# vlongle/pixie

Hardware: AMD Instinct MI355X
Metric: voxels/s (128^3 U-Net fwd) + MPM particle-steps/s (higher is better)
Workload: dtype f32 (operands split fp16 hi+lo, 3 f16 MFMAs/product, fp32 accumulate); 1 GPU; 128^3x64 feature grid -> SegmentationUNet+RegressionUNet forward (+argmax/one-hot combine), 1 scene per GPU per step; grid=128, feature_channels=64, parallelism=scene-parallel x1, executor=c+hip_graph

## Files before the change

### pixie_amd/csrc/conv3d_f16x3.hip

```cpp
#include <hip/hip_runtime.h>

#include <cstdlib>
#include <map>
#include <string>
#include <type_traits>

#include "../../include/pixie_hip.h"
#include "common.h"

namespace pixie {

typedef float f32x16 __attribute__((ext_vector_type(16)));
typedef _Float16 f16x8 __attribute__((ext_vector_type(8)));

constexpr int kW16HeaderU4 = 4;

struct Conv16Args {
    const float* in0; const float* in1;
    int c0, cin;
    int ID, IH, IW;
    int LD, LH, LW;
    int ups;
    int stride;
    int OD, OH, OW;
    const float* pro_a; const float* pro_b; const float* gamma; const float* beta;
    int act;
    const uint4* w16;
    const float* wf;
    const float* bias;
    int cout, coutp;
    const float* residual; float* out;
    const unsigned* amax0; const unsigned* amax1;
    float in_bound;
    int TX, TY, TZ, lTX, lTY;
    int tiles_x, tiles_y, tiles_z, n_tiles;
    int HX, HY, HZ, HYX, CS;
    unsigned mHX, mHYX;
    float* stats; unsigned* out_amax;
    float* partial; int chunks_per_slice;
    int epi_lds;
    const float* sk_in0; const float* sk_in1;
    int sk_c0, sk_cin;
    const uint4* sk_w16; const float* sk_bias;
    const unsigned* sk_amax0; const unsigned* sk_amax1;
};

__device__ __forceinline__ int fast_div16(int n, int d, unsigned magic) {
    return (d == 1) ? n : (int)__umulhi((unsigned)n, magic);
}
__device__ __forceinline__ float act16(float t, int act) {
    if (act == 1) return t > 0.0f ? t : 0.02f * t;
    if (act == 2) return t / (1.0f + __expf(-t));
    return t;
}
__device__ __forceinline__ int scale_exponent(float bound) {
    const unsigned bits = __float_as_uint(bound);
    const int eb = (int)((bits >> 23) & 0xffu) - 127;
    if (!(bound > 0.0f) || eb > 100) return 0;
    int e = 14 - eb;
    return e > 100 ? 100 : (e < -100 ? -100 : e);
}
__device__ __forceinline__ float pow2i(int e) { return __uint_as_float((unsigned)(e + 127) << 23); }

template <int KS, int MB, int NB, bool EX = false, bool SP = false>
__device__ __forceinline__ void conv3d_f16x3_body(const Conv16Args& A) {
    static_assert(!SP || (KS == 3 && NB == 4 && !EX), "sub-pixel path: 3^3, two x parities x two voxel blocks per wave");
    extern __shared__ uint4 smem16[];
    constexpr int PAD = (KS == 3) ? 1 : 0;
    constexpr int NW = 4, NT = 64 * NW;
    const int bufsz = 4 * A.CS;

    const int tid = threadIdx.x;
    const int lane = tid & 63;
    const int wave = tid >> 6;
    const int kh = lane >> 5;
    const int l31 = lane & 31;

    int t = blockIdx.x;
    {
        const int per = (A.n_tiles + 7) >> 3;
        const int cand = (t & 7) * per + (t >> 3);
        if ((A.n_tiles & 7) == 0) t = cand;
    }
    int par = 0;
    if constexpr (SP) { par = t & 3; t >>= 2; }
    const int py = par & 1, pz = par >> 1;
    const int tx = t % A.tiles_x; t /= A.tiles_x;
    const int ty = t % A.tiles_y;
    const int tz = t / A.tiles_y;
    const int ox0 = tx * A.TX, oy0 = ty * A.TY, oz0 = tz * A.TZ;
    const int cout0 = blockIdx.y * (MB * 32);
    const int lx0 = SP ? ox0 - 1 : ox0 * A.stride - PAD;
    const int ly0 = SP ? oy0 - 1 + py : oy0 * A.stride - PAD;
    const int lz0 = SP ? oz0 - 1 + pz : oz0 * A.stride - PAD;
    const size_t ISP = (size_t)A.ID * A.IH * A.IW;
    const size_t OSP = (size_t)A.OD * A.OH * A.OW;

    int voff[NB];
    int ovox[NB];
    bool valid[NB];
#pragma unroll
    for (int nb = 0; nb < NB; ++nb) {
        if constexpr (SP) {
            const int px = nb >> 1;
            const int j = (wave * 2 + (nb & 1)) * 32 + l31;
            int x = j & (A.TX - 1);
            int y = (j >> A.lTX) & (A.TY - 1);
            int z = j >> (A.lTX + A.lTY);
            const int gx = 2 * (ox0 + x) + px, gy = 2 * (oy0 + y) + py, gz = 2 * (oz0 + z) + pz;
            const bool v = (z < A.TZ) && (gx < A.OW) && (gy < A.OH) && (gz < A.OD);
            if (!v) { x = 0; y = 0; z = 0; }
            voff[nb] = (z * A.HY + y) * A.HX + x + px + kh * A.CS;
            ovox[nb] = v ? (gz * A.OH + gy) * A.OW + gx : 0;
            valid[nb] = v;
            continue;
        }
        const int j = (wave * NB + nb) * 32 + l31;
        int x = j & (A.TX - 1);
        int y = (j >> A.lTX) & (A.TY - 1);
        int z = j >> (A.lTX + A.lTY);
        const bool v = (z < A.TZ) && (ox0 + x < A.OW) && (oy0 + y < A.OH) && (oz0 + z < A.OD);
        if (!v) { x = 0; y = 0; z = 0; }
        voff[nb] = ((z * A.HY + y) * A.HX + x) * A.stride + kh * A.CS;
        ovox[nb] = ((oz0 + z) * A.OH + (oy0 + y)) * A.OW + ox0 + x;
        valid[nb] = v;
    }

    float bound = A.in_bound;
    if (A.amax0) {
        bound = __uint_as_float(*A.amax0);
        if (A.amax1) bound = fmaxf(bound, __uint_as_float(*A.amax1));
    }
    const int ex = EX ? 0 : scale_exponent(bound);
    const float sx = pow2i(ex);

    f32x16 acc[MB][NB];
#pragma unroll
    for (int mb = 0; mb < MB; ++mb)
#pragma unroll
        for (int nb = 0; nb < NB; ++nb)
#pragma unroll
            for (int r = 0; r < 16; ++r) acc[mb][nb][r] = 0.0f;

    const int KG = A.cin >> 3;
    const size_t tap_stride = (size_t)KG * A.coutp;
    const size_t plane = (size_t)(SP ? 64 : KS * KS * KS) * tap_stride;
    const uint4* wHi = A.w16 + kW16HeaderU4 + (size_t)kh * A.coutp + cout0 + l31 + (size_t)(par * 16) * tap_stride;
    const uint4* wLo = wHi + plane;
    const float* wF = A.wf + (size_t)kh * A.coutp + cout0 + l31;

    constexpr int TAPS = KS * KS * KS;
    auto stage_chunk = [&](int c_base, uint4* buf, int stid, int nthr) {
        uint4* bHi = buf;
        uint4* bLo = buf + 2 * A.CS;
        float pa[16], pb[16];
        {
            float pv = 0.0f;
            if (A.pro_a) pv = (lane & 16) ? A.pro_b[c_base + (lane & 15)] : A.pro_a[c_base + (lane & 15)];
#pragma unroll
            for (int j = 0; j < 16; ++j) {
                pa[j] = __int_as_float(__builtin_amdgcn_readlane(__float_as_int(pv), j));
                pb[j] = __int_as_float(__builtin_amdgcn_readlane(__float_as_int(pv), 16 + j));
            }
        }
        const bool has_aff = A.gamma != nullptr;
        for (int v0 = stid; v0 < A.CS; v0 += 2 * nthr) {
            float val[2][16];
            float gm[2], bt[2];
            int sidx[2];
            bool ok[2];
#pragma unroll
            for (int u = 0; u < 2; ++u) {
                const int vox = v0 + u * nthr;
                int rem = vox;
                const int hz = fast_div16(rem, A.HYX, A.mHYX);
                rem -= hz * A.HYX;
                const int hy = fast_div16(rem, A.HX, A.mHX);
                const int hx = rem - hy * A.HX;
                const int lz = lz0 + hz, ly = ly0 + hy, lx = lx0 + hx;
                ok[u] = vox < A.CS && (unsigned)lz < (unsigned)A.LD && (unsigned)ly < (unsigned)A.LH && (unsigned)lx < (unsigned)A.LW;
                sidx[u] = ok[u] ? ((lz >> A.ups) * A.IH + (ly >> A.ups)) * A.IW + (lx >> A.ups) : 0;
            }
#pragma unroll
            for (int u = 0; u < 2; ++u) {
#pragma unroll
                for (int j = 0; j < 16; ++j) {
                    const int cg = c_base + j;
                    const float* src = (cg < A.c0) ? (A.in0 + (size_t)cg * ISP) : (A.in1 + (size_t)(cg - A.c0) * ISP);
                    val[u][j] = src[sidx[u]];
                }
                gm[u] = 1.0f; bt[u] = 0.0f;
                if (has_aff) { gm[u] = A.gamma[sidx[u]]; bt[u] = A.beta[sidx[u]]; }
            }
            auto convert = [&](auto has_pro, auto act_c) {
#pragma unroll
                for (int u = 0; u < 2; ++u) {
                    const int vox = v0 + u * nthr;
                    if (EX) {
                        float* bF = reinterpret_cast<float*>(buf);
#pragma unroll
                        for (int j = 0; j < 16; ++j) {
                            float t = val[u][j];
                            if (decltype(has_pro)::value) t = t * pa[j] + pb[j];
                            t = t * gm[u] + bt[u];
                            const float sc = ok[u] ? act16(t, decltype(act_c)::value) : 0.0f;
                            if (vox < A.CS) bF[j * A.CS + vox] = sc;
                        }
                        continue;
                    }
                    f16x8 vh[2], vl[2];
#pragma unroll
                    for (int j = 0; j < 16; ++j) {
                        float t = val[u][j];
                        if (decltype(has_pro)::value) t = t * pa[j] + pb[j];
                        t = t * gm[u] + bt[u];
                        const float sc = ok[u] ? act16(t, decltype(act_c)::value) * sx : 0.0f;
                        const _Float16 h = (_Float16)sc;
                        vh[j >> 3][j & 7] = h;
                        vl[j >> 3][j & 7] = (_Float16)(sc - (float)h);
                    }
                    if (vox < A.CS) {
                        bHi[vox] = __builtin_bit_cast(uint4, vh[0]);
                        bHi[A.CS + vox] = __builtin_bit_cast(uint4, vh[1]);
                        bLo[vox] = __builtin_bit_cast(uint4, vl[0]);
                        bLo[A.CS + vox] = __builtin_bit_cast(uint4, vl[1]);
                    }
                }
            };
            using T = std::true_type; using F = std::false_type;
            if (A.pro_a) {
                if (A.act == 1) convert(T{}, std::integral_constant<int, 1>{});
                else if (A.act == 2) convert(T{}, std::integral_constant<int, 2>{});
                else convert(T{}, std::integral_constant<int, 0>{});
            } else {
                if (A.act == 1) convert(F{}, std::integral_constant<int, 1>{});
                else if (A.act == 2) convert(F{}, std::integral_constant<int, 2>{});
                else convert(F{}, std::integral_constant<int, 0>{});
            }
        }
    };
    auto mfma_chunk = [&](int c_base, const uint4* buf) {
        __builtin_amdgcn_s_setprio(3);
        if constexpr (EX) {
            const float* ldsF = reinterpret_cast<const float*>(buf);
            const size_t tapw = (size_t)A.cin * A.coutp;
            const float* wc = wF + (size_t)c_base * A.coutp;
            float a[8][MB], an[8][MB];
#pragma unroll
            for (int kp = 0; kp < 8; ++kp)
#pragma unroll
                for (int mb = 0; mb < MB; ++mb) a[kp][mb] = wc[(size_t)(2 * kp) * A.coutp + mb * 32];
#pragma unroll 1
            for (int zy = 0; zy < KS * KS; ++zy) {
                const int dz = zy / KS, dy = zy - dz * KS;
                const int rowoff = (dz * A.HY + dy) * A.HX;
#pragma unroll
                for (int dx = 0; dx < KS; ++dx) {
                    const int tap = zy * KS + dx;
                    const int nxt = (tap + 1 < TAPS) ? tap + 1 : tap;
#pragma unroll
                    for (int kp = 0; kp < 8; ++kp)
#pragma unroll
                        for (int mb = 0; mb < MB; ++mb) an[kp][mb] = wc[(size_t)nxt * tapw + (size_t)(2 * kp) * A.coutp + mb * 32];
                    __builtin_amdgcn_sched_barrier(0);
#pragma unroll
                    for (int kp = 0; kp < 8; ++kp) {
                        float b[NB];
#pragma unroll
                        for (int nb = 0; nb < NB; ++nb) b[nb] = ldsF[voff[nb] + rowoff + dx + 2 * kp * A.CS];
#pragma unroll
                        for (int mb = 0; mb < MB; ++mb)
#pragma unroll
                            for (int nb = 0; nb < NB; ++nb)
                                acc[mb][nb] = __builtin_amdgcn_mfma_f32_32x32x2f32(a[kp][mb], b[nb], acc[mb][nb], 0, 0, 0);
                    }
#pragma unroll
                    for (int kp = 0; kp < 8; ++kp)
#pragma unroll
                        for (int mb = 0; mb < MB; ++mb) a[kp][mb] = an[kp][mb];
                }
            }
            __builtin_amdgcn_s_setprio(0);
            return;
        }
        const uint4* ldsHi = buf;
        const uint4* ldsLo = buf + 2 * A.CS;
        const uint4* wh = wHi + (size_t)(c_base >> 3) * A.coutp;
        const uint4* wl = wLo + (size_t)(c_base >> 3) * A.coutp;
        if constexpr (SP) {
            f16x8 ah[MB], al[MB];
#pragma unroll
            for (int mb = 0; mb < MB; ++mb) {
                ah[mb] = __builtin_bit_cast(f16x8, wh[mb * 32]);
                al[mb] = __builtin_bit_cast(f16x8, wl[mb * 32]);
            }
#pragma unroll 1
            for (int zy = 0; zy < 4; ++zy) {
                const int rowoff = ((zy >> 1) * A.HY + (zy & 1)) * A.HX;
                const int zyn = zy < 3 ? zy + 1 : 3;
#pragma unroll
                for (int q = 0; q < 4; ++q) {
                    const int ex = q >> 1, px = q & 1;
                    const size_t nxt = (q < 3) ? (size_t)(((q + 1) & 1) * 8 + zy * 2 + ((q + 1) >> 1)) * tap_stride : (size_t)(zyn * 2) * tap_stride;
                    f16x8 ahn[MB], aln[MB];
#pragma unroll
                    for (int mb = 0; mb < MB; ++mb) {
                        ahn[mb] = __builtin_bit_cast(f16x8, wh[nxt + mb * 32]);
                        aln[mb] = __builtin_bit_cast(f16x8, wl[nxt + mb * 32]);
                    }
                    __builtin_amdgcn_sched_barrier(0);
                    f16x8 bh[2], bl[2];
#pragma unroll
                    for (int s = 0; s < 2; ++s) {
                        bh[s] = __builtin_bit_cast(f16x8, ldsHi[voff[px * 2 + s] + rowoff + ex]);
                        bl[s] = __builtin_bit_cast(f16x8, ldsLo[voff[px * 2 + s] + rowoff + ex]);
                    }
#pragma unroll
                    for (int mb = 0; mb < MB; ++mb)
#pragma unroll
                        for (int s = 0; s < 2; ++s)
                            acc[mb][px * 2 + s] = __builtin_amdgcn_mfma_f32_32x32x16_f16(al[mb], bh[s], acc[mb][px * 2 + s], 0, 0, 0);
#pragma unroll
                    for (int mb = 0; mb < MB; ++mb)
#pragma unroll
                        for (int s = 0; s < 2; ++s)
                            acc[mb][px * 2 + s] = __builtin_amdgcn_mfma_f32_32x32x16_f16(ah[mb], bl[s], acc[mb][px * 2 + s], 0, 0, 0);
#pragma unroll
                    for (int mb = 0; mb < MB; ++mb)
#pragma unroll
                        for (int s = 0; s < 2; ++s)
                            acc[mb][px * 2 + s] = __builtin_amdgcn_mfma_f32_32x32x16_f16(ah[mb], bh[s], acc[mb][px * 2 + s], 0, 0, 0);
#pragma unroll
                    for (int mb = 0; mb < MB; ++mb) { ah[mb] = ahn[mb]; al[mb] = aln[mb]; }
                }
            }
            __builtin_amdgcn_s_setprio(0);
            return;
        }
        f16x8 ah[MB], al[MB];
#pragma unroll
        for (int mb = 0; mb < MB; ++mb) {
            ah[mb] = __builtin_bit_cast(f16x8, wh[mb * 32]);
            al[mb] = __builtin_bit_cast(f16x8, wl[mb * 32]);
        }
#pragma unroll 1
        for (int zy = 0; zy < KS * KS; ++zy) {
            const int dz = zy / KS, dy = zy - dz * KS;
            const int rowoff = (dz * A.HY + dy) * A.HX;
#pragma unroll
            for (int dx = 0; dx < KS; ++dx) {
                const int tap = zy * KS + dx;
                const int nxt = (tap + 1 < TAPS) ? tap + 1 : tap;
                f16x8 ahn[MB], aln[MB];
#pragma unroll
                for (int mb = 0; mb < MB; ++mb) {
                    ahn[mb] = __builtin_bit_cast(f16x8, wh[(size_t)nxt * tap_stride + mb * 32]);
                    aln[mb] = __builtin_bit_cast(f16x8, wl[(size_t)nxt * tap_stride + mb * 32]);
                }
                __builtin_amdgcn_sched_barrier(0);
                f16x8 bh[NB], bl[NB];
#pragma unroll
                for (int nb = 0; nb < NB; ++nb) {
                    bh[nb] = __builtin_bit_cast(f16x8, ldsHi[voff[nb] + rowoff + dx]);
                    bl[nb] = __builtin_bit_cast(f16x8, ldsLo[voff[nb] + rowoff + dx]);
                }
#pragma unroll
                for (int mb = 0; mb < MB; ++mb)
#pragma unroll
                    for (int nb = 0; nb < NB; ++nb)
                        acc[mb][nb] = __builtin_amdgcn_mfma_f32_32x32x16_f16(al[mb], bh[nb], acc[mb][nb], 0, 0, 0);
#pragma unroll
                for (int mb = 0; mb < MB; ++mb)
#pragma unroll
                    for (int nb = 0; nb < NB; ++nb)
                        acc[mb][nb] = __builtin_amdgcn_mfma_f32_32x32x16_f16(ah[mb], bl[nb], acc[mb][nb], 0, 0, 0);
#pragma unroll
                for (int mb = 0; mb < MB; ++mb)
#pragma unroll
                    for (int nb = 0; nb < NB; ++nb)
                        acc[mb][nb] = __builtin_amdgcn_mfma_f32_32x32x16_f16(ah[mb], bh[nb], acc[mb][nb], 0, 0, 0);
#pragma unroll
                for (int mb = 0; mb < MB; ++mb) { ah[mb] = ahn[mb]; al[mb] = aln[mb]; }
            }
        }
        __builtin_amdgcn_s_setprio(0);
    };

    float inv2 = 0.0f;
    {
        const int c_begin = A.partial ? (int)blockIdx.z * A.chunks_per_slice * 16 : 0;
        const int c_end = A.partial ? min(A.cin, c_begin + A.chunks_per_slice * 16) : A.cin;
        for (int c_base = c_begin; c_base < c_end; c_base += 16) {
            __syncthreads();
            stage_chunk(c_base, smem16, tid, NT);
            __syncthreads();
            mfma_chunk(c_base, smem16);
        }
        if (!EX && !SP && A.sk_w16) {
            float sb = __uint_as_float(*A.sk_amax0);
            if (A.sk_amax1) sb = fmaxf(sb, __uint_as_float(*A.sk_amax1));
            const int ex2 = scale_exponent(sb);
            const float sx2 = pow2i(ex2);
            const float inv_main = __uint_as_float(A.w16[0].x) * pow2i(-ex);
            inv2 = __uint_as_float(A.sk_w16[0].x) * pow2i(-ex2);
            const float ratio = inv_main / inv2;
#pragma unroll
            for (int mb = 0; mb < MB; ++mb)
#pragma unroll
                for (int nb = 0; nb < NB; ++nb)
#pragma unroll
                    for (int r = 0; r < 16; ++r) acc[mb][nb][r] *= ratio;
            const int KG2 = A.sk_cin >> 3;
            const uint4* w2Hi = A.sk_w16 + kW16HeaderU4 + (size_t)kh * A.coutp + cout0 + l31;
            const uint4* w2Lo = w2Hi + (size_t)KG2 * A.coutp;
            const int centre = (KS == 3) ? (A.HY + 1) * A.HX + 1 : 0;
            const int tvox = A.TX * A.TY * A.TZ;
            for (int c2 = 0; c2 < A.sk_cin; c2 += 16) {
                f16x8 ah[MB], al[MB];
#pragma unroll
                for (int mb = 0; mb < MB; ++mb) {
                    ah[mb] = __builtin_bit_cast(f16x8, w2Hi[(size_t)(c2 >> 3) * A.coutp + mb * 32]);
                    al[mb] = __builtin_bit_cast(f16x8, w2Lo[(size_t)(c2 >> 3) * A.coutp + mb * 32]);
                }
                __syncthreads();
                uint4* bHi = smem16;
                uint4* bLo = smem16 + 2 * A.CS;
                for (int j = tid; j < tvox; j += NT) {
                    const int x = j & (A.TX - 1), y = (j >> A.lTX) & (A.TY - 1), z = j >> (A.lTX + A.lTY);
                    const bool okv = (ox0 + x < A.OW) && (oy0 + y < A.OH) && (oz0 + z < A.OD);
                    const size_t sidx = okv ? ((size_t)(oz0 + z) * A.IH + (oy0 + y)) * A.IW + ox0 + x : 0;
                    float val[16];
#pragma unroll
                    for (int q = 0; q < 16; ++q) {
                        const int cg = c2 + q;
                        const float* src = (cg < A.sk_c0) ? (A.sk_in0 + (size_t)cg * ISP) : (A.sk_in1 + (size_t)(cg - A.sk_c0) * ISP);
                        val[q] = src[sidx];
                    }
                    f16x8 vh[2], vl[2];
#pragma unroll
                    for (int q = 0; q < 16; ++q) {
                        const float sc = okv ? val[q] * sx2 : 0.0f;
                        const _Float16 hq = (_Float16)sc;
                        vh[q >> 3][q & 7] = hq;
                        vl[q >> 3][q & 7] = (_Float16)(sc - (float)hq);
                    }
                    const int slot = (z * A.HY + y) * A.HX + x + centre;
                    bHi[slot] = __builtin_bit_cast(uint4, vh[0]);
                    bHi[A.CS + slot] = __builtin_bit_cast(uint4, vh[1]);
                    bLo[slot] = __builtin_bit_cast(uint4, vl[0]);
                    bLo[A.CS + slot] = __builtin_bit_cast(uint4, vl[1]);
                }
                __syncthreads();
                f16x8 bh[NB], bl[NB];
#pragma unroll
                for (int nb = 0; nb < NB; ++nb) {
                    bh[nb] = __builtin_bit_cast(f16x8, bHi[voff[nb] + centre]);
                    bl[nb] = __builtin_bit_cast(f16x8, bLo[voff[nb] + centre]);
                }
#pragma unroll
                for (int mb = 0; mb < MB; ++mb)
#pragma unroll
                    for (int nb = 0; nb < NB; ++nb)
                        acc[mb][nb] = __builtin_amdgcn_mfma_f32_32x32x16_f16(al[mb], bh[nb], acc[mb][nb], 0, 0, 0);
#pragma unroll
                for (int mb = 0; mb < MB; ++mb)
#pragma unroll
                    for (int nb = 0; nb < NB; ++nb)
                        acc[mb][nb] = __builtin_amdgcn_mfma_f32_32x32x16_f16(ah[mb], bl[nb], acc[mb][nb], 0, 0, 0);
#pragma unroll
                for (int mb = 0; mb < MB; ++mb)
#pragma unroll
                    for (int nb = 0; nb < NB; ++nb)
                        acc[mb][nb] = __builtin_amdgcn_mfma_f32_32x32x16_f16(ah[mb], bh[nb], acc[mb][nb], 0, 0, 0);
            }
        }
    }

    const float inv = EX ? 1.0f : (A.sk_w16 ? inv2 : __uint_as_float(A.w16[0].x) * pow2i(-ex));
    if (A.partial) {
        float* dst = A.partial + (size_t)blockIdx.z * A.cout * OSP;
#pragma unroll
        for (int mb = 0; mb < MB; ++mb)
#pragma unroll
            for (int r = 0; r < 16; ++r) {
                const int co = cout0 + mb * 32 + (r & 3) + 8 * (r >> 2) + 4 * kh;
                if (co < A.cout) {
#pragma unroll
                    for (int nb = 0; nb < NB; ++nb)
                        if (valid[nb]) dst[(size_t)co * OSP + ovox[nb]] = acc[mb][nb][r] * inv;
                }
            }
        return;
    }
    float* red = reinterpret_cast<float*>(smem16);
    float wmax = 0.0f;
    const bool full = SP ? (A.epi_lds && cout0 + MB * 32 <= A.cout && (A.TX & 1) == 0 && (A.OW & 3) == 0 && NW * 64 <= A.TX * A.TY * A.TZ &&
                            2 * (ox0 + A.TX) <= A.OW && 2 * (oy0 + A.TY) <= A.OH && 2 * (oz0 + A.TZ) <= A.OD)
                         : (A.epi_lds && cout0 + MB * 32 <= A.cout && (A.TX & 3) == 0 && (A.OW & 3) == 0 && NW * NB * 32 <= A.TX * A.TY * A.TZ &&
                            ox0 + A.TX <= A.OW && oy0 + A.TY <= A.OH && oz0 + A.TZ <= A.OD);
    if (full) {
        __syncthreads();
        constexpr int LDO = NB * 32 + 4;
        float* ldsO = reinterpret_cast<float*>(smem16) + wave * (32 * LDO);
        red = reinterpret_cast<float*>(smem16) + NW * 32 * LDO;
        constexpr int LPR = NB * 8;
        constexpr int RPI = 32 / LPR;
        const int rsub = l31 / LPR, colq = 4 * (l31 % LPR), nbq = colq >> 5;
        const int jq = SP ? wave * 64 + (colq >> 1) : (wave * NB + nbq) * 32 + (colq & 31);
        const int xq = jq & (A.TX - 1), yq = (jq >> A.lTX) & (A.TY - 1), zq = jq >> (A.lTX + A.lTY);
        const size_t ovq = SP ? ((size_t)(2 * (oz0 + zq) + pz) * A.OH + (2 * (oy0 + yq) + py)) * A.OW + 2 * (ox0 + xq)
                              : ((size_t)(oz0 + zq) * A.OH + (oy0 + yq)) * A.OW + ox0 + xq;
        const bool has_res = A.residual != nullptr, has_stats = A.stats != nullptr;
#pragma unroll
        for (int mb = 0; mb < MB; ++mb) {
#pragma unroll
            for (int r = 0; r < 16; ++r)
#pragma unroll
                for (int nb = 0; nb < NB; ++nb)
                    ldsO[((r & 3) + 8 * (r >> 2) + 4 * kh) * LDO + (SP ? 2 * ((nb & 1) * 32 + l31) + (nb >> 1) : nb * 32 + l31)] = acc[mb][nb][r];
#pragma unroll 4
            for (int it = 0; it < 16 / RPI; ++it) {
                const int rowl = (2 * it + kh) * RPI + rsub;
                const int co = cout0 + mb * 32 + rowl;
                const float4 a4 = *reinterpret_cast<const float4*>(ldsO + rowl * LDO + colq);
                const float bv = (A.bias ? A.bias[co] : 0.0f) + (A.sk_bias ? A.sk_bias[co] : 0.0f);
                const size_t o = (size_t)co * OSP + ovq;
                float4 v4;
                v4.x = a4.x * inv + bv; v4.y = a4.y * inv + bv; v4.z = a4.z * inv + bv; v4.w = a4.w * inv + bv;
                if (has_res) {
                    const float4 r4 = *reinterpret_cast<const float4*>(A.residual + o);
                    v4.x += r4.x; v4.y += r4.y; v4.z += r4.z; v4.w += r4.w;
                }
                *reinterpret_cast<float4*>(A.out + o) = v4;
                if (has_stats) {
                    float s1 = (v4.x + v4.y) + (v4.z + v4.w);
                    float s2 = (v4.x * v4.x + v4.y * v4.y) + (v4.z * v4.z + v4.w * v4.w);
                    wmax = fmaxf(fmaxf(wmax, fmaxf(fabsf(v4.x), fabsf(v4.y))), fmaxf(fabsf(v4.z), fabsf(v4.w)));
#pragma unroll
                    for (int off = LPR / 2; off > 0; off >>= 1) { s1 += __shfl_xor(s1, off, 64); s2 += __shfl_xor(s2, off, 64); }
                    if ((l31 % LPR) == 0) { red[(wave * MB * 32 + mb * 32 + rowl) * 2] = s1; red[(wave * MB * 32 + mb * 32 + rowl) * 2 + 1] = s2; }
                }
            }
        }
    } else {
    if (A.stats) __syncthreads();
#pragma unroll
    for (int mb = 0; mb < MB; ++mb) {
#pragma unroll
        for (int r = 0; r < 16; ++r) {
            const int row = mb * 32 + (r & 3) + 8 * (r >> 2) + 4 * kh;
            const int co = cout0 + row;
            float s1 = 0.0f, s2 = 0.0f;
            if (co < A.cout) {
                const float bv = (A.bias ? A.bias[co] : 0.0f) + (A.sk_bias ? A.sk_bias[co] : 0.0f);
#pragma unroll
                for (int nb = 0; nb < NB; ++nb) {
                    if (valid[nb]) {
                        const size_t o = (size_t)co * OSP + ovox[nb];
                        float val = acc[mb][nb][r] * inv + bv;
                        if (A.residual) val += A.residual[o];
                        A.out[o] = val;
                        s1 += val; s2 += val * val; wmax = fmaxf(wmax, fabsf(val));
                    }
                }
            }
            if (A.stats) {
#pragma unroll
                for (int off = 16; off > 0; off >>= 1) { s1 += __shfl_xor(s1, off, 64); s2 += __shfl_xor(s2, off, 64); }
                if (l31 == 0) { red[(wave * MB * 32 + row) * 2] = s1; red[(wave * MB * 32 + row) * 2 + 1] = s2; }
            }
        }
    }
    }
    if (A.stats) {
        __syncthreads();
        if (tid < MB * 32 * 2) {
            float t = red[tid];
#pragma unroll
            for (int w = 1; w < NW; ++w) t += red[w * MB * 64 + tid];
            A.stats[((size_t)blockIdx.x * A.coutp + cout0) * 2 + tid] = t;
        }
        if (A.out_amax) {
#pragma unroll
            for (int off = 32; off > 0; off >>= 1) wmax = fmaxf(wmax, __shfl_xor(wmax, off, 64));
            if (lane == 0 && wmax > 0.0f) atomicMax(A.out_amax, __float_as_uint(wmax));
        }
    }
}

template <int KS, int MB, int NB>
__global__ __launch_bounds__(256, 2) void conv3d_f16x3_kernel(Conv16Args A) {
    conv3d_f16x3_body<KS, MB, NB>(A);
}
template <int KS, int MB, int NB>
__global__ __launch_bounds__(256, 2) void conv3d_exact_kernel(Conv16Args A) {
    conv3d_f16x3_body<KS, MB, NB, true>(A);
}
template <int MB>
__global__ __launch_bounds__(256, 2) void conv3d_f16x3_subpixel_kernel(Conv16Args A) {
    conv3d_f16x3_body<3, MB, 4, false, true>(A);
}
__global__ __launch_bounds__(256, 2) void conv3d_f16x3_c64_fullres_kernel(Conv16Args A) {
    conv3d_f16x3_body<3, 2, 4>(A);
}

struct StatParts { const void* p; int n; long cstride, tstride; int f64; };

__device__ inline void block_channel_sums(const StatParts& P, int c, double* r, double& o1, double& o2) {
    double s1 = 0.0, s2 = 0.0;
    for (int t = threadIdx.x; t < P.n; t += 256) {
        const size_t k = ((size_t)c * P.cstride + (size_t)t * P.tstride) * 2;
        if (P.f64) { const double2 v = *reinterpret_cast<const double2*>(static_cast<const double*>(P.p) + k); s1 += v.x; s2 += v.y; }
        else { const float2 v = *reinterpret_cast<const float2*>(static_cast<const float*>(P.p) + k); s1 += v.x; s2 += v.y; }
    }
    for (int off = 32; off > 0; off >>= 1) { s1 += __shfl_down(s1, off, 64); s2 += __shfl_down(s2, off, 64); }
    if ((threadIdx.x & 63) == 0) { r[2 * (threadIdx.x >> 6)] = s1; r[2 * (threadIdx.x >> 6) + 1] = s2; }
    __syncthreads();
    o1 = r[0] + r[2] + r[4] + r[6]; o2 = r[1] + r[3] + r[5] + r[7];
    __syncthreads();
}

__global__ __launch_bounds__(256) void stats_finalize_kernel(StatParts P, double* __restrict__ sums) {
    const int c = blockIdx.x;
    __shared__ double r[8];
    double s1, s2;
    block_channel_sums(P, c, r, s1, s2);
    if (threadIdx.x == 0) { sums[2 * c] = s1; sums[2 * c + 1] = s2; }
}

__global__ __launch_bounds__(256) void stats_norm_finalize_kernel(StatParts P0, double* sums0, int c0, StatParts P1, double* sums1, int channels,
                                                                  double spatial, int mode, int groups, double eps,
                                                                  const float* __restrict__ weight, const float* __restrict__ bias,
                                                                  float* __restrict__ a, float* __restrict__ b) {
    __shared__ double r[8];
    const int cpg = mode == 0 ? 1 : channels / groups;
    const int first = blockIdx.x * cpg;
    double s1 = 0.0, s2 = 0.0;
    for (int k = first; k < first + cpg; ++k) {
        const bool in0 = k < c0;
        const StatParts& P = in0 ? P0 : P1;
        double* sums = in0 ? sums0 : sums1;
        const int kc = in0 ? k : k - c0;
        double t1, t2;
        if (P.n > 0) {
            block_channel_sums(P, kc, r, t1, t2);
            if (threadIdx.x == 0) { sums[2 * kc] = t1; sums[2 * kc + 1] = t2; }
        } else {
            t1 = sums[2 * kc]; t2 = sums[2 * kc + 1];
        }
        s1 += t1; s2 += t2;
    }
    const double cnt = mode == 0 ? spatial : spatial * cpg;
    const double mean = s1 / cnt;
    double var = s2 / cnt - mean * mean;
    if (var < 0.0) var = 0.0;
    const double rstd = 1.0 / sqrt(var + eps);
    for (int k = first + threadIdx.x; k < first + cpg; k += 256) {
        if (mode == 0) {
            a[k] = (float)rstd;
            b[k] = (float)(-mean * rstd);
        } else {
            const double w = weight ? (double)weight[k] : 1.0;
            const double bb = bias ? (double)bias[k] : 0.0;
            a[k] = (float)(rstd * w);
            b[k] = (float)(bb - mean * rstd * w);
        }
    }
}

__global__ __launch_bounds__(256) void splitk_reduce_kernel(const float* __restrict__ partial, int slices, long n_elems, long osp,
                                                            const float* __restrict__ bias, const float* residual, float* out) {
    const long i = (long)blockIdx.x * 256 + threadIdx.x;
    if (i >= n_elems) return;
    float v = partial[i];
    for (int s = 1; s < slices; ++s) v += partial[(size_t)s * n_elems + i];
    if (bias) v += bias[i / osp];
    if (residual) v += residual[i];
    out[i] = v;
}

constexpr int kReduceSeg = 4096;
template <bool VEC>
__global__ __launch_bounds__(256) void splitk_reduce_stats_kernel(const float* __restrict__ partial, int slices, long n_elems, long osp,
                                                                  const float* __restrict__ bias, const float* residual, float* out,
                                                                  double* __restrict__ stats, unsigned* out_amax) {
    const int c = blockIdx.y;
    const long seg0 = (long)blockIdx.x * kReduceSeg;
    const size_t base = (size_t)c * osp;
    const float bv = bias ? bias[c] : 0.0f;
    double s1 = 0.0, s2 = 0.0;
    float mx = 0.0f;
    if (VEC) {
#pragma unroll
        for (int k = 0; k < kReduceSeg / 1024; ++k) {
            const long j = seg0 + k * 1024 + (long)threadIdx.x * 4;
            if (j < osp) {
                const size_t i = base + j;
                float4 v = *reinterpret_cast<const float4*>(partial + i);
                for (int s = 1; s < slices; ++s) {
                    const float4 q = *reinterpret_cast<const float4*>(partial + (size_t)s * n_elems + i);
                    v.x += q.x; v.y += q.y; v.z += q.z; v.w += q.w;
                }
                if (bias) { v.x += bv; v.y += bv; v.z += bv; v.w += bv; }
                if (residual) {
                    const float4 q = *reinterpret_cast<const float4*>(residual + i);
                    v.x += q.x; v.y += q.y; v.z += q.z; v.w += q.w;
                }
                *reinterpret_cast<float4*>(out + i) = v;
                const double x = v.x, y = v.y, z = v.z, w = v.w;
                s1 += (x + y) + (z + w);
                s2 += (x * x + y * y) + (z * z + w * w);
                mx = fmaxf(fmaxf(mx, fmaxf(fabsf(v.x), fabsf(v.y))), fmaxf(fabsf(v.z), fabsf(v.w)));
            }
        }
    } else {
#pragma unroll 4
        for (int k = 0; k < kReduceSeg / 256; ++k) {
            const long j = seg0 + k * 256 + threadIdx.x;
            if (j < osp) {
                const size_t i = base + j;
                float v = partial[i];
                for (int s = 1; s < slices; ++s) v += partial[(size_t)s * n_elems + i];
                if (bias) v += bv;
                if (residual) v += residual[i];
                out[i] = v;
                const double x = v;
                s1 += x; s2 += x * x; mx = fmaxf(mx, fabsf(v));
            }
        }
    }
    for (int off = 32; off > 0; off >>= 1) {
        s1 += __shfl_down(s1, off, 64);
        s2 += __shfl_down(s2, off, 64);
        mx = fmaxf(mx, __shfl_down(mx, off, 64));
    }
    __shared__ double r[8];
    __shared__ float rmx[4];
    const int lane = threadIdx.x & 63, wave = threadIdx.x >> 6;
    if (lane == 0) { r[2 * wave] = s1; r[2 * wave + 1] = s2; rmx[wave] = mx; }
    __syncthreads();
    if (threadIdx.x == 0) {
        double* dst = stats + ((size_t)c * gridDim.x + blockIdx.x) * 2;
        dst[0] = r[0] + r[2] + r[4] + r[6];
        dst[1] = r[1] + r[3] + r[5] + r[7];
        const unsigned m = __float_as_uint(fmaxf(fmaxf(rmx[0], rmx[1]), fmaxf(rmx[2], rmx[3])));
        if (out_amax && m > __hip_atomic_load(out_amax, __ATOMIC_RELAXED, __HIP_MEMORY_SCOPE_AGENT)) atomicMax(out_amax, m);
    }
}

__global__ __launch_bounds__(256) void amax_kernel(const float* __restrict__ x, long n, unsigned* __restrict__ slot) {
    float m = 0.0f;
    const long stride = (long)gridDim.x * 256 * 4;
    long i = ((long)blockIdx.x * 256 + threadIdx.x) * 4;
    if ((reinterpret_cast<size_t>(x) & 15) == 0) {
        for (; i + 3 < n; i += stride) {
            const float4 v = *reinterpret_cast<const float4*>(x + i);
            m = fmaxf(fmaxf(m, fabsf(v.x)), fmaxf(fabsf(v.y), fmaxf(fabsf(v.z), fabsf(v.w))));
        }
        for (long k = i; k < n && k < i + 4; ++k) m = fmaxf(m, fabsf(x[k]));
    } else {
        for (long k = (long)blockIdx.x * 256 + threadIdx.x; k < n; k += (long)gridDim.x * 256) m = fmaxf(m, fabsf(x[k]));
    }
    for (int off = 32; off > 0; off >>= 1) m = fmaxf(m, __shfl_down(m, off, 64));
    if ((threadIdx.x & 63) == 0 && m > 0.0f) atomicMax(slot, __float_as_uint(m));
}

__global__ void pack_weights_f16x2_kernel(const float* __restrict__ src, uint4* __restrict__ dst, int cout, int cin, int taps,
                                          int coutp, const unsigned* __restrict__ amax_bits) {
    const int KG = cin >> 3;
    const long total = (long)taps * KG * coutp;
    const long i = (long)blockIdx.x * blockDim.x + threadIdx.x;
    const int e = scale_exponent(__uint_as_float(*amax_bits));
    if (i == 0) dst[0] = make_uint4(__float_as_uint(pow2i(-e)), (unsigned)cout, (unsigned)cin, (unsigned)taps);
    if (i >= total) return;
    const float s = pow2i(e);
    const int co = (int)(i % coutp);
    const long row = i / coutp;
    const int kg = (int)(row % KG);
    const int tap = (int)(row / KG);
    f16x8 vh, vl;
#pragma unroll
    for (int j = 0; j < 8; ++j) {
        float w = 0.0f;
        if (co < cout) w = src[((long)co * cin + kg * 8 + j) * taps + tap] * s;
        const _Float16 h = (_Float16)w;
        vh[j] = h;
        vl[j] = (_Float16)(w - (float)h);
    }
    dst[kW16HeaderU4 + i] = __builtin_bit_cast(uint4, vh);
    dst[kW16HeaderU4 + total + i] = __builtin_bit_cast(uint4, vl);
}

__device__ __forceinline__ float subpixel_weight(const float* __restrict__ w27, int par, int tap) {
    int lo[3], hi[3];
#pragma unroll
    for (int ax = 0; ax < 3; ++ax) {
        const int p = (par >> (2 - ax)) & 1, e = (tap >> (2 - ax)) & 1;
        lo[ax] = e ? (p ? 2 : 1) : 0;
        hi[ax] = e ? 2 : (p ? 1 : 0);
    }
    float sum = 0.0f;
    for (int dz = lo[0]; dz <= hi[0]; ++dz)
        for (int dy = lo[1]; dy <= hi[1]; ++dy)
            for (int dx = lo[2]; dx <= hi[2]; ++dx) sum += w27[(dz * 3 + dy) * 3 + dx];
    return sum;
}
__global__ __launch_bounds__(256) void subpixel_amax_kernel(const float* __restrict__ src, long pairs, unsigned* __restrict__ slot) {
    const long i = (long)blockIdx.x * 256 + threadIdx.x;
    float m = 0.0f;
    if (i < pairs)
        for (int pt = 0; pt < 64; ++pt) m = fmaxf(m, fabsf(subpixel_weight(src + i * 27, pt >> 3, pt & 7)));
    for (int off = 32; off > 0; off >>= 1) m = fmaxf(m, __shfl_down(m, off, 64));
    if ((threadIdx.x & 63) == 0 && m > 0.0f) atomicMax(slot, __float_as_uint(m));
}
__global__ void pack_weights_subpixel_kernel(const float* __restrict__ src, uint4* __restrict__ dst, int cout, int cin, int coutp,
                                             const unsigned* __restrict__ amax_bits) {
    const int KG = cin >> 3;
    const long total = 64L * KG * coutp;
    const long i = (long)blockIdx.x * blockDim.x + threadIdx.x;
    const int e = scale_exponent(__uint_as_float(*amax_bits));
    if (i == 0) dst[0] = make_uint4(__float_as_uint(pow2i(-e)), (unsigned)cout, (unsigned)cin, 64u);
    if (i >= total) return;
    const float s = pow2i(e);
    const int co = (int)(i % coutp);
    const long row = i / coutp;
    const int kg = (int)(row % KG);
    const int pt = (int)(row / KG);
    f16x8 vh, vl;
#pragma unroll
    for (int j = 0; j < 8; ++j) {
        float w = 0.0f;
        if (co < cout) w = subpixel_weight(src + ((long)co * cin + kg * 8 + j) * 27, pt >> 3, pt & 7) * s;
        const _Float16 h = (_Float16)w;
        vh[j] = h;
        vl[j] = (_Float16)(w - (float)h);
    }
    dst[kW16HeaderU4 + i] = __builtin_bit_cast(uint4, vh);
    dst[kW16HeaderU4 + total + i] = __builtin_bit_cast(uint4, vl);
}

static unsigned magic_of16(int d) { return d <= 1 ? 0u : (unsigned)((0x100000000ull + (unsigned long long)d - 1) / (unsigned long long)d); }
static int ilog2_16(int v) { int l = 0; while ((1 << l) < v) ++l; return l; }
static int pow2_le16(int v, int cap) { int p = 1; while (p * 2 <= v && p * 2 <= cap) p *= 2; return p; }

template <int MB>
static int launch_subpixel(const Conv16Args& a, size_t lds_bytes, dim3 grid, hipStream_t st) {
    auto kern = conv3d_f16x3_subpixel_kernel<MB>;
    PX_CHECK_HIP(allow_max_dynamic_lds(reinterpret_cast<const void*>(kern)));
    hipLaunchKernelGGL(kern, grid, dim3(256), lds_bytes, st, a);
    PX_CHECK_HIP(hipGetLastError());
    return 0;
}

static bool conv16_subpixel(const pixie_conv_desc* d) {
    return d->d_w16 && d->w16_subpixel && d->upsample == 1 && d->ksize == 3 && d->stride == 1;
}

template <int KS, int MB, int NB>
static int launch_f16x3(const Conv16Args& a, size_t lds_bytes, dim3 grid, hipStream_t st) {
    auto kern = conv3d_f16x3_kernel<KS, MB, NB>;
    PX_CHECK_HIP(allow_max_dynamic_lds(reinterpret_cast<const void*>(kern)));
    hipLaunchKernelGGL(kern, grid, dim3(256), lds_bytes, st, a);
    PX_CHECK_HIP(hipGetLastError());
    return 0;
}

static void conv16_tiling(const pixie_conv_desc* d, Conv16Args& a, int& MB_out, int& NB_out, int* slices_out = nullptr) {
    a.ID = d->in_d; a.IH = d->in_h; a.IW = d->in_w;
    a.ups = d->upsample;
    a.LD = a.ID << a.ups; a.LH = a.IH << a.ups; a.LW = a.IW << a.ups;
    const int pad = d->ksize == 3 ? 1 : 0;
    a.stride = d->stride;
    a.OD = (a.LD + 2 * pad - d->ksize) / a.stride + 1; a.OH = (a.LH + 2 * pad - d->ksize) / a.stride + 1; a.OW = (a.LW + 2 * pad - d->ksize) / a.stride + 1;
    if (d->out_d > 0) a.OD = std::min(a.OD, (int)d->out_d);
    if (d->out_h > 0) a.OH = std::min(a.OH, (int)d->out_h);
    if (d->out_w > 0) a.OW = std::min(a.OW, (int)d->out_w);
    a.cout = d->c_out; a.coutp = pixie_conv_cout_padded(d->c_out);
    const int chunks = (d->c0 + d->c1) / 16;
    const int smax = d->d_workspace ? std::min(8, chunks / 2) : 1;
    if (conv16_subpixel(d)) {
        a.ups = 0; a.LD = a.ID; a.LH = a.IH; a.LW = a.IW;
        const int SD = (a.OD + 1) / 2, SH = (a.OH + 1) / 2, SW = (a.OW + 1) / 2;
        a.TX = pow2_le16(SW, 32);
        a.TY = pow2_le16(SH, std::max(1, std::min(4, 256 / a.TX)));
        a.TZ = std::max(1, std::min(SD, 256 / (a.TX * a.TY)));
        a.lTX = ilog2_16(a.TX); a.lTY = ilog2_16(a.TY);
        a.tiles_x = (SW + a.TX - 1) / a.TX; a.tiles_y = (SH + a.TY - 1) / a.TY; a.tiles_z = (SD + a.TZ - 1) / a.TZ;
        a.n_tiles = 4 * a.tiles_x * a.tiles_y * a.tiles_z;
        a.HX = a.TX + 2; a.HY = a.TY + 1; a.HZ = a.TZ + 1;
        a.HYX = a.HY * a.HX; a.CS = a.HZ * a.HYX;
        a.mHX = magic_of16(a.HX); a.mHYX = magic_of16(a.HYX);
        MB_out = (a.coutp >= 64) ? 2 : 1; NB_out = 4;
        int sl = 1;
        const long wgs = (long)a.n_tiles * ((a.coutp + MB_out * 32 - 1) / (MB_out * 32));
        while (sl * 2 <= smax && wgs * sl < 512) sl *= 2;
        if (slices_out) *slices_out = sl;
        return;
    }
    const long ovol = (long)a.OD * a.OH * a.OW;
    int MB = (a.coutp >= 64) ? 2 : 1;
    int NB = (a.stride == 2) ? 1 : 4;
    auto n_wg = [&](int mb, int nb) {
        const long tiles = (ovol + 128L * nb - 1) / (128L * nb);
        return tiles * ((a.coutp + mb * 32 - 1) / (mb * 32));
    };
    int slices = 1;
    if (smax >= 2 && n_wg(MB, NB) < 512) {
        bool found = false;
        for (int nb = NB; nb >= 1 && !found; nb /= 2) {
            for (int sl = 1; sl <= smax; sl *= 2)
                if (n_wg(MB, nb) * sl >= 512) { NB = nb; slices = sl; found = true; break; }
        }
        if (!found) { NB = 1; slices = 1; while (slices * 2 <= smax) slices *= 2; }
    } else {
        while (n_wg(MB, NB) < 512 && NB > 1) NB /= 2;
        if (n_wg(MB, NB) < 512 && MB > 1) MB = 1;
    }
    if (slices_out) *slices_out = slices;
    const int tile_vox = 128 * NB;
    a.TX = pow2_le16(a.OW, 32);
    a.TY = pow2_le16(a.OH, std::max(1, std::min(4, tile_vox / a.TX)));
    a.TZ = std::max(1, std::min(a.OD, tile_vox / (a.TX * a.TY)));
    a.lTX = ilog2_16(a.TX); a.lTY = ilog2_16(a.TY);
    a.tiles_x = (a.OW + a.TX - 1) / a.TX; a.tiles_y = (a.OH + a.TY - 1) / a.TY; a.tiles_z = (a.OD + a.TZ - 1) / a.TZ;
    a.n_tiles = a.tiles_x * a.tiles_y * a.tiles_z;
    a.HX = (a.TX - 1) * a.stride + d->ksize; a.HY = (a.TY - 1) * a.stride + d->ksize; a.HZ = (a.TZ - 1) * a.stride + d->ksize;
    a.HYX = a.HY * a.HX; a.CS = a.HZ * a.HYX;
    a.mHX = magic_of16(a.HX); a.mHYX = magic_of16(a.HYX);

    MB_out = MB; NB_out = NB;
}

static int reduce_segments(long osp) { return (int)((osp + kReduceSeg - 1) / kReduceSeg); }

static StatParts conv16_stat_parts(const pixie_conv_desc* d, const void* stats) {
    Conv16Args a{};
    int MB = 0, NB = 0, slices = 1;
    conv16_tiling(d, a, MB, NB, &slices);
    if (slices > 1) {
        const int n = reduce_segments((long)a.OD * a.OH * a.OW);
        return StatParts{stats, n, n, 1, 1};
    }
// ... 110 lines not shown
    PX_CHECK_HIP(allow_max_dynamic_lds(reinterpret_cast<const void*>(kern)));
    hipLaunchKernelGGL(kern, grid, dim3(256), lds_bytes, st, a);
    PX_CHECK_HIP(hipGetLastError());
    return 0;
}

bool conv3d_exact_tiled_ok(const pixie_conv_desc* d) {
    const int cin = d->c0 + d->c1;
    return cin % 16 == 0 && (d->stride == 1 || (d->stride == 2 && d->ksize == 3 && !d->upsample)) && getenv("PIXIE_CONV_EXACT_V1") == nullptr;
}

int conv3d_exact_forward(const pixie_conv_desc* d, hipStream_t st) {
    Conv16Args a{};
    a.in0 = d->d_in0; a.in1 = d->d_in1; a.c0 = d->c0; a.cin = d->c0 + d->c1;
    a.pro_a = d->d_pro_a; a.pro_b = d->d_pro_b; a.gamma = d->d_gamma; a.beta = d->d_beta; a.act = d->act;
    a.wf = d->d_w; a.bias = d->d_bias;
    a.residual = d->d_residual; a.out = d->d_out;
    a.in_bound = 1.0f;
    int MB = 0, NB = 0;
    conv16_exact_tiling(d, a, MB, NB);
    size_t lds = (size_t)4 * a.CS * sizeof(uint4);
    PX_REQUIRE(lds <= 160 * 1024, "exact conv: tile needs %zu B of LDS", lds);
    if (conv16_epi_lds(MB, NB, 1)) { a.epi_lds = 1; lds = std::max(lds, conv16_epi_bytes(MB, NB)); }
    const dim3 grid((unsigned)a.n_tiles, (unsigned)((a.coutp + MB * 32 - 1) / (MB * 32)), 1u);
#define PX_CONVEX_CASE(KS_, MB_, NB_) \
    if (d->ksize == KS_ && MB == MB_ && NB == NB_) return launch_exact<KS_, MB_, NB_>(a, lds, grid, st);
    PX_CONVEX_CASE(3, 2, 4) PX_CONVEX_CASE(3, 2, 2) PX_CONVEX_CASE(3, 2, 1)
    PX_CONVEX_CASE(3, 1, 4) PX_CONVEX_CASE(3, 1, 2) PX_CONVEX_CASE(3, 1, 1)
    PX_CONVEX_CASE(1, 2, 4) PX_CONVEX_CASE(1, 2, 2) PX_CONVEX_CASE(1, 2, 1)
    PX_CONVEX_CASE(1, 1, 4) PX_CONVEX_CASE(1, 1, 2) PX_CONVEX_CASE(1, 1, 1)
#undef PX_CONVEX_CASE
    return set_error("exact conv: no kernel variant for ksize=%d MB=%d NB=%d", d->ksize, MB, NB);
}

}

using namespace pixie;

extern "C" int64_t pixie_conv_stats_floats(const pixie_conv_desc* d) {
    if (!d || !d->d_w16 || !(d->stride == 1 || (d->stride == 2 && d->ksize == 3)) || (d->ksize != 1 && d->ksize != 3)) return 0;
    Conv16Args a{};
    int MB = 0, NB = 0, slices = 1;
    conv16_tiling(d, a, MB, NB, &slices);
    if (slices > 1) return (int64_t)a.cout * reduce_segments((long)a.OD * a.OH * a.OW) * 2 * (int64_t)(sizeof(double) / sizeof(float));
    return (int64_t)a.n_tiles * a.coutp * 2;
}

extern "C" int64_t pixie_conv_workspace_bytes(const pixie_conv_desc* d) {
    if (!d || !d->d_w16 || !(d->stride == 1 || (d->stride == 2 && d->ksize == 3)) || (d->ksize != 1 && d->ksize != 3)) return 0;
    pixie_conv_desc probe = *d;
    probe.d_workspace = reinterpret_cast<void*>(1);
    Conv16Args a{};
    int MB = 0, NB = 0, slices = 1;
    conv16_tiling(&probe, a, MB, NB, &slices);
    return slices > 1 ? (int64_t)slices * a.cout * a.OD * a.OH * a.OW * (int64_t)sizeof(float) : 0;
}

#ifdef PIXIE_DIAG
extern "C" int pixie_conv_kernel_variant(const pixie_conv_desc* d, int* slices_out) {
    if (slices_out) *slices_out = 1;
    if (!d || !d->d_w16 || !(d->stride == 1 || (d->stride == 2 && d->ksize == 3)) || (d->ksize != 1 && d->ksize != 3)) return 0;
    Conv16Args a{};
    int MB = 0, NB = 0, slices = 1;
    conv16_tiling(d, a, MB, NB, &slices);
    if (slices_out) *slices_out = slices;
    if (conv16_subpixel(d)) return 8300 + MB * 10 + NB;
    if (d->ksize == 3 && MB == 2 && NB == 4 && d->c0 + d->c1 == 64 && d->c_out == 64 && d->stride == 1 && !d->upsample && d->c1 == 0 && !d->d_skip_w16 &&
        (long)a.OD * a.OH * a.OW >= 128L * 128 * 128)
        return 9324;
    return d->ksize * 100 + MB * 10 + NB;
}

extern "C" int pixie_conv_tile_geometry(const pixie_conv_desc* d, int32_t out[10]) {
    if (!d || !out || (d->ksize != 1 && d->ksize != 3) || !(d->stride == 1 || (d->stride == 2 && d->ksize == 3 && !d->upsample))) return 1;
    if ((d->c0 + d->c1) % 16 != 0 || (d->d_w16 && d->c0 % 8 != 0)) return 1;
    if (!d->d_w16 && !conv3d_exact_tiled_ok(d)) return 1;
    Conv16Args a{};
    int MB = 0, NB = 0, slices = 1;
    if (d->d_w16) conv16_tiling(d, a, MB, NB, &slices);
    else conv16_exact_tiling(d, a, MB, NB);
    const int32_t v[10] = {a.TX, a.TY, a.TZ, a.tiles_x, a.tiles_y, a.tiles_z, conv16_epi_lds(MB, NB, slices) ? 1 : 0, slices, MB, NB};
    for (int i = 0; i < 10; ++i) out[i] = v[i];
    return 0;
}

extern "C" int pixie_conv_stats_layout(const pixie_conv_desc* d, int64_t out[6]) {
    if (!out || pixie_conv_stats_floats(d) <= 0) return 1;
    const StatParts p = conv16_stat_parts(d, nullptr);
    out[0] = p.n; out[1] = p.cstride; out[2] = p.tstride; out[3] = p.f64; out[4] = p.f64 ? kReduceSeg : 0;
    out[5] = pixie_conv_cout_padded(d->c_out);
    return 0;
}
#endif

extern "C" int pixie_conv_skip_foldable(const pixie_conv_desc* d) {
    if (!d || !d->d_w16 || d->stride != 1 || d->upsample || (d->ksize != 1 && d->ksize != 3)) return 0;
    const int scin = d->skip_c0 + d->skip_c1;
    if (scin <= 0 || scin % 16 != 0 || d->skip_c0 % 8 != 0 || (d->c0 + d->c1) % 16 != 0 || d->c0 % 8 != 0) return 0;
    Conv16Args a{};
    int MB = 0, NB = 0, slices = 1;
    conv16_tiling(d, a, MB, NB, &slices);
    return slices == 1 ? 1 : 0;
}

extern "C" int pixie_stats_finalize(const float* d_stats, const pixie_conv_desc* d, double* d_sums, void* stream) {
    PX_REQUIRE(d_stats && d && d_sums, "pixie_stats_finalize: null argument");
    hipLaunchKernelGGL(stats_finalize_kernel, dim3((unsigned)d->c_out), dim3(256), 0, as_stream(stream), conv16_stat_parts(d, d_stats), d_sums);
    PX_CHECK_HIP(hipGetLastError());
    return 0;
}

extern "C" int pixie_stats_norm_finalize(const float* d_stats0, const pixie_conv_desc* desc0, double* d_sums0, const float* d_stats1,
                                         const pixie_conv_desc* desc1, double* d_sums1, int c1, int64_t spatial, int mode, int groups,
                                         double eps, const float* d_weight, const float* d_bias, float* d_a, float* d_b, void* stream) {
    PX_REQUIRE(desc0 && d_sums0 && d_a && d_b && spatial > 0 && c1 >= 0, "pixie_stats_norm_finalize: bad arguments");
    PX_REQUIRE(c1 == 0 || d_sums1, "pixie_stats_norm_finalize: a second part needs d_sums1");
    PX_REQUIRE(!d_stats1 || desc1, "pixie_stats_norm_finalize: d_stats1 needs its descriptor");
    const int c0 = desc0->c_out, channels = c0 + c1;
    PX_REQUIRE(!d_stats1 || desc1->c_out == c1, "pixie_stats_norm_finalize: desc1 has %d output channels, c1 is %d", desc1 ? desc1->c_out : 0, c1);
    PX_REQUIRE(mode == 0 || (mode == 1 && groups > 0 && channels % groups == 0), "pixie_stats_norm_finalize: bad mode/groups");
    const StatParts none{nullptr, 0, 0, 0, 0};
    const StatParts p0 = d_stats0 ? conv16_stat_parts(desc0, d_stats0) : none;
    const StatParts p1 = d_stats1 ? conv16_stat_parts(desc1, d_stats1) : none;
    hipLaunchKernelGGL(stats_norm_finalize_kernel, dim3((unsigned)(mode == 0 ? channels : groups)), dim3(256), 0, as_stream(stream), p0, d_sums0, c0,
                       p1, d_sums1, channels, (double)spatial, mode, groups, eps, d_weight, d_bias, d_a, d_b);
    PX_CHECK_HIP(hipGetLastError());
    return 0;
}

extern "C" int64_t pixie_conv_packed16_bytes(int c_out, int c_in, int ksize) {
    if (c_out <= 0 || c_in <= 0 || c_in % 8 != 0 || (ksize != 1 && ksize != 3)) return 0;
    const int64_t taps = (int64_t)ksize * ksize * ksize;
    return ((int64_t)kW16HeaderU4 + 2 * taps * (c_in / 8) * pixie_conv_cout_padded(c_out)) * (int64_t)sizeof(uint4);
}

extern "C" int pixie_tensor_amax(const float* d_x, int64_t count, uint32_t* d_slot, void* stream) {
    PX_REQUIRE(d_x && d_slot && count > 0, "pixie_tensor_amax: bad arguments");
    const int blocks = (int)std::min<int64_t>(2048, (count + 1023) / 1024);
    hipLaunchKernelGGL(amax_kernel, dim3(blocks), dim3(256), 0, as_stream(stream), d_x, (long)count, d_slot);
    PX_CHECK_HIP(hipGetLastError());
    return 0;
}

extern "C" int pixie_conv_pack_weights_f16x2(const float* d_w, void* d_packed, int c_out, int c_in, int ksize, void* stream) {
    PX_REQUIRE(d_w && d_packed && c_out > 0 && c_in > 0 && c_in % 8 == 0 && (ksize == 1 || ksize == 3),
               "pixie_conv_pack_weights_f16x2: bad arguments (c_in must be a multiple of 8)");
    hipStream_t st = as_stream(stream);
    const int taps = ksize * ksize * ksize;
    const int coutp = pixie_conv_cout_padded(c_out);
    unsigned* slot = reinterpret_cast<unsigned*>(d_packed) + 15;
    PX_CHECK_HIP(hipMemsetAsync(d_packed, 0, kW16HeaderU4 * sizeof(uint4), st));
    if (pixie_tensor_amax(d_w, (int64_t)c_out * c_in * taps, slot, stream)) return 1;
    const long total = (long)taps * (c_in / 8) * coutp;
    hipLaunchKernelGGL(pack_weights_f16x2_kernel, dim3(cdiv(total, 256)), dim3(256), 0, st, d_w, reinterpret_cast<uint4*>(d_packed), c_out,
                       c_in, taps, coutp, slot);
    PX_CHECK_HIP(hipGetLastError());
    return 0;
}

extern "C" int64_t pixie_conv_subpixel_bytes(int c_out, int c_in) {
    if (c_out <= 0 || c_in <= 0 || c_in % 16 != 0) return 0;
    return ((int64_t)kW16HeaderU4 + 2 * 64 * (int64_t)(c_in / 8) * pixie_conv_cout_padded(c_out)) * (int64_t)sizeof(uint4);
}

extern "C" int pixie_conv_pack_weights_subpixel(const float* d_w, void* d_packed, int c_out, int c_in, void* stream) {
    PX_REQUIRE(d_w && d_packed && c_out > 0 && c_in > 0 && c_in % 16 == 0,
               "pixie_conv_pack_weights_subpixel: bad arguments (c_in must be a multiple of 16)");
    hipStream_t st = as_stream(stream);
    const int coutp = pixie_conv_cout_padded(c_out);
    unsigned* slot = reinterpret_cast<unsigned*>(d_packed) + 15;
    PX_CHECK_HIP(hipMemsetAsync(d_packed, 0, kW16HeaderU4 * sizeof(uint4), st));
    const long pairs = (long)c_out * c_in;
    hipLaunchKernelGGL(subpixel_amax_kernel, dim3(cdiv(pairs, 256)), dim3(256), 0, st, d_w, pairs, slot);
    PX_CHECK_HIP(hipGetLastError());
    const long total = 64L * (c_in / 8) * coutp;
    hipLaunchKernelGGL(pack_weights_subpixel_kernel, dim3(cdiv(total, 256)), dim3(256), 0, st, d_w, reinterpret_cast<uint4*>(d_packed), c_out,
                       c_in, coutp, slot);
    PX_CHECK_HIP(hipGetLastError());
    return 0;
}
```

Baseline: 24.37 million voxels/s.

## Row-pack hi/lo weight halves for small-cout 3x3x3 head convolutions

After: 24.35 million voxels/s. About the same (-0.1%).

```diff
diff --git a/pixie_amd/csrc/conv3d_f16x3.hip b/pixie_amd/csrc/conv3d_f16x3.hip
--- a/pixie_amd/csrc/conv3d_f16x3.hip
+++ b/pixie_amd/csrc/conv3d_f16x3.hip
@@ -14,6 +14,8 @@
 typedef _Float16 f16x8 __attribute__((ext_vector_type(8)));
 
 constexpr int kW16HeaderU4 = 4;
+constexpr unsigned kW16Plain = 0u, kW16RowPacked = 1u;
+constexpr int kRowPackMaxCout = 8;
 
 struct Conv16Args {
     const float* in0; const float* in1;
@@ -134,6 +136,10 @@
     const int ex = EX ? 0 : scale_exponent(bound);
     const float sx = pow2i(ex);
 
+    constexpr bool RP = KS == 3 && MB == 1 && NB == 4 && !EX && !SP;
+    bool rowpack = false;
+    if constexpr (RP) rowpack = A.w16[1].x == kW16RowPacked && !A.sk_w16;
+
     f32x16 acc[MB][NB];
 #pragma unroll
     for (int mb = 0; mb < MB; ++mb)
@@ -337,6 +343,38 @@
             __builtin_amdgcn_s_setprio(0);
             return;
         }
+        if constexpr (RP) {
+            if (rowpack) {
+                f16x8 a = __builtin_bit_cast(f16x8, wh[0]);
+#pragma unroll 1
+                for (int zy = 0; zy < KS * KS; ++zy) {
+                    const int dz = zy / KS, dy = zy - dz * KS;
+                    const int rowoff = (dz * A.HY + dy) * A.HX;
+#pragma unroll
+                    for (int dx = 0; dx < KS; ++dx) {
+                        const int tap = zy * KS + dx;
+                        const int nxt = (tap + 1 < TAPS) ? tap + 1 : tap;
+                        const f16x8 an = __builtin_bit_cast(f16x8, wh[(size_t)nxt * tap_stride]);
+                        __builtin_amdgcn_sched_barrier(0);
+                        f16x8 bh[NB], bl[NB];
+#pragma unroll
+                        for (int nb = 0; nb < NB; ++nb) {
+                            bh[nb] = __builtin_bit_cast(f16x8, ldsHi[voff[nb] + rowoff + dx]);
+                            bl[nb] = __builtin_bit_cast(f16x8, ldsLo[voff[nb] + rowoff + dx]);
+                        }
+#pragma unroll
+                        for (int nb = 0; nb < NB; ++nb)
+                            acc[0][nb] = __builtin_amdgcn_mfma_f32_32x32x16_f16(a, bl[nb], acc[0][nb], 0, 0, 0);
+#pragma unroll
+                        for (int nb = 0; nb < NB; ++nb)
+                            acc[0][nb] = __builtin_amdgcn_mfma_f32_32x32x16_f16(a, bh[nb], acc[0][nb], 0, 0, 0);
+                        a = an;
+                    }
+                }
+                __builtin_amdgcn_s_setprio(0);
+                return;
+            }
+        }
         f16x8 ah[MB], al[MB];
 #pragma unroll
         for (int mb = 0; mb < MB; ++mb) {
@@ -473,6 +511,15 @@
                     for (int nb = 0; nb < NB; ++nb)
                         acc[mb][nb] = __builtin_amdgcn_mfma_f32_32x32x16_f16(ah[mb], bh[nb], acc[mb][nb], 0, 0, 0);
             }
+        }
+    }
+
+    if constexpr (RP) {
+        if (rowpack) {
+#pragma unroll
+            for (int nb = 0; nb < NB; ++nb)
+#pragma unroll
+                for (int r = 0; r < 4; ++r) acc[0][nb][r] += acc[0][nb][r + 4];
         }
     }
 
@@ -766,28 +813,36 @@
 }
 
 __global__ void pack_weights_f16x2_kernel(const float* __restrict__ src, uint4* __restrict__ dst, int cout, int cin, int taps,
-                                          int coutp, const unsigned* __restrict__ amax_bits) {
+                                          int coutp, const unsigned* __restrict__ amax_bits, unsigned form) {
     const int KG = cin >> 3;
     const long total = (long)taps * KG * coutp;
     const long i = (long)blockIdx.x * blockDim.x + threadIdx.x;
     const int e = scale_exponent(__uint_as_float(*amax_bits));
-    if (i == 0) dst[0] = make_uint4(__float_as_uint(pow2i(-e)), (unsigned)cout, (unsigned)cin, (unsigned)taps);
+    if (i == 0) {
+        dst[0] = make_uint4(__float_as_uint(pow2i(-e)), (unsigned)cout, (unsigned)cin, (unsigned)taps);
+        dst[1] = make_uint4(form, 0u, 0u, 0u);
+    }
     if (i >= total) return;
     const float s = pow2i(e);
     const int co = (int)(i % coutp);
     const long row = i / coutp;
     const int kg = (int)(row % KG);
     const int tap = (int)(row / KG);
+    const bool twin = form == kW16RowPacked && co >= kRowPackMaxCout && co < 2 * kRowPackMaxCout;
+    const int cs = twin ? co - kRowPackMaxCout : co;
     f16x8 vh, vl;
 #pragma unroll
     for (int j = 0; j < 8; ++j) {
         float w = 0.0f;
-        if (co < cout) w = src[((long)co * cin + kg * 8 + j) * taps + tap] * s;
+        if (cs < cout) w = src[((long)cs * cin + kg * 8 + j) * taps + tap] * s;
         const _Float16 h = (_Float16)w;
         vh[j] = h;
         vl[j] = (_Float16)(w - (float)h);
     }
-    dst[kW16HeaderU4 + i] = __builtin_bit_cast(uint4, vh);
+    dst[kW16HeaderU4 + i] = __builtin_bit_cast(uint4, twin ? vl : vh);
+    if (twin)
+#pragma unroll
+        for (int j = 0; j < 8; ++j) vl[j] = (_Float16)0.0f;
     dst[kW16HeaderU4 + total + i] = __builtin_bit_cast(uint4, vl);
 }
 
@@ -1204,8 +1259,10 @@
     PX_CHECK_HIP(hipMemsetAsync(d_packed, 0, kW16HeaderU4 * sizeof(uint4), st));
     if (pixie_tensor_amax(d_w, (int64_t)c_out * c_in * taps, slot, stream)) return 1;
     const long total = (long)taps * (c_in / 8) * coutp;
+    const char* rp = getenv("PIXIE_HEAD_ROWPACK");
+    const unsigned form = (ksize == 3 && c_out <= kRowPackMaxCout && coutp >= 2 * kRowPackMaxCout && !(rp && rp[0] == '0')) ? kW16RowPacked : kW16Plain;
     hipLaunchKernelGGL(pack_weights_f16x2_kernel, dim3(cdiv(total, 256)), dim3(256), 0, st, d_w, reinterpret_cast<uint4*>(d_packed), c_out,
-                       c_in, taps, coutp, slot);
+                       c_in, taps, coutp, slot, form);
     PX_CHECK_HIP(hipGetLastError());
     return 0;
 }
```
